# xujiabo/SCREAM

Hardware: AMD Instinct MI355X
Metric: registration pairs/sec (higher is better)
Workload: dtype f32; 1 GPU; BASELINE configs[1]: synthetic 3DMatch_test-like pairs, voxel 0.0625 m, ~5k points/cloud, batch-of-pairs=32 per GPU, A1-A10 per pair (forward 6+6 layers d_model 256, 1-NN thresh 0.1, Kabsch, RE/TE), random-init weights seed 0; lanes=1, steps_in_flight=2, parallelism=dp1 (pairs sharded, metric-row all-gather), rccl_ranks=1, gemm_backend=h2

## Files before the change

### scream_amd/csrc/proj_ring.hip

```cpp
#include <type_traits>

#include "matrix_front.h"
#include "ring.h"

namespace {

constexpr int P_PF = 2;
constexpr int P_LB = 2;

constexpr int P_KV_ELEMS = (SCREAM_HEAD_DIM + 1) * SCREAM_HEAD_DIM;
constexpr int P_SLAB_BYTES = 4 * P_KV_ELEMS * 4;

struct ProjArgs {
    const float* x;
    const char* Wimg;
    float* Q;
    int64_t M;
    int32_t n_q;
    int32_t S;
    float* kv_partial;
    int64_t kv_layer_stride;
    const int32_t* tile_cloud;
    const int32_t* cloud_row0;
    const int32_t* cloud_len;
    int64_t row_base;
    float a_scale, kv_sk, kv_cv, kv_inv;
    Elu1Consts ec;
};

template <class SP>
__global__ __launch_bounds__(TT, 1) void proj_ring_kernel(ProjArgs pa) {
    typedef typename SP::vec V;
    constexpr int NP = SP::NP;
    constexpr int STAGE = stage_bytes<SP>();
    constexpr int PIECES = wave_pieces<SP>();
    constexpr int INFLIGHT = PIECES;
    constexpr int GM = 2 * SP::NPROD;
    constexpr int Q_WIN = 12;
    constexpr int PIECE_STRIDE = (15 - Q_WIN) * GM / PIECES;
    static_assert(PIECE_STRIDE >= 1, "the groups behind the stores hold the stage's pieces");
    __shared__ __attribute__((aligned(16))) char smem[T_SLOTS * STAGE + P_SLAB_BYTES];
    float* slabs = reinterpret_cast<float*>(smem + T_SLOTS * STAGE);
    const int tid = threadIdx.x, lane = tid & 63;
    const int wave = __builtin_amdgcn_readfirstlane(tid >> 6);
    const int half = lane >> 5, r = lane & 31;
    const unsigned v_lane16 = lane * 16;

    const int S = pa.S, UPT = S >> 1, nq2 = pa.n_q >> 1;
    const int64_t n_tiles = (pa.M + 255) >> 8;
    const int64_t U = n_tiles * UPT;
    const int64_t u_lo = U * blockIdx.x / gridDim.x, u_hi = U * (blockIdx.x + 1) / gridDim.x;
    if (u_lo >= u_hi) return;
    const int s0 = (int)(u_lo % UPT) * 2;

    unsigned q = 0;
    auto dma_piece = [&](unsigned qq, int u) __attribute__((always_inline)) {
        const unsigned img = (unsigned)(s0 + qq) % (unsigned)S, slot = qq % (unsigned)T_SLOTS;
        const char* sbase = pa.Wimg + (size_t)img * STAGE + (wave * PIECES + (u & ~3)) * 1024;
        dma_1k(sbase + v_lane16, smem + slot * STAGE + (wave * PIECES + (u & ~3)) * 1024, u & 3);
    };
#pragma unroll
    for (int u = 0; u < PIECES; ++u) dma_piece(0, u);
#pragma unroll
    for (int u = 0; u < PIECES; ++u) dma_piece(1, u);

    V xp[2][16][NP];
    int64_t tile = -1;
    bool wave_ok = false;
    int valid0 = 0;
    float* part_tile = nullptr;
    float* qg = nullptr;

    auto enter_tile = [&](int64_t t) __attribute__((always_inline)) {
        tile = t;
        const int64_t t128 = t * 2 + (wave >> 1);
        wave_ok = t128 * 128 < pa.M;
        const int64_t row0 = wave_ok ? t * 256 + wave * 64 : t * 256;
        const float* g = pa.x + row0 * SCREAM_D_MODEL + lane * 4;
        valid0 = 0;
        if (wave_ok && pa.S > pa.n_q) {
            const int64_t arow = pa.row_base + t128 * 128;
            const int cloud = pa.tile_cloud[arow / SCREAM_ROW_TILE];
            valid0 = pa.cloud_len[cloud] - (int)(arow - pa.cloud_row0[cloud]) - (wave & 1) * 64;
        }
        part_tile = pa.kv_partial + t128 * SCREAM_NHEAD * P_KV_ELEMS;
        qg = pa.Q + row0 * SCREAM_D_MODEL + lane * 4;
        constexpr int LB = P_LB, NB = 16 / LB;
        f32x4 raw[2][LB][4];
        auto request = [&](int b) __attribute__((always_inline)) {
            const int rg = b / (NB / 2), blk0 = LB * (b % (NB / 2));
#pragma unroll
            for (int k = 0; k < LB; ++k)
#pragma unroll
                for (int a = 0; a < 4; ++a)
                    raw[b & 1][k][a] = __builtin_nontemporal_load(reinterpret_cast<const f32x4*>(g + rg * 8192 + ((blk0 + k) * 4 + a) * 256));
        };
        request(0);
#pragma unroll
        for (int b = 0; b < NB; ++b) {
            const int rg = b / (NB / 2), blk0 = LB * (b % (NB / 2));
            __builtin_amdgcn_sched_barrier(0);
            if (b + 1 < NB) request(b + 1);
            __builtin_amdgcn_sched_barrier(0);
#pragma unroll
            for (int k = 0; k < LB; ++k)
#pragma unroll
                for (int s2 = 0; s2 < 2; ++s2)
                {
                    V tmp[NP];
#pragma unroll
                    for (int j = 0; j < 8; ++j) SP::split1s(raw[b & 1][k][2 * s2 + (j >> 2)][j & 3], pa.a_scale, j, tmp);
#pragma unroll
                    for (int p = 0; p < NP; ++p) {
                        asm volatile("" : "+a"(tmp[p]));
                        xp[rg][2 * (blk0 + k) + s2][p] = tmp[p];
                    }
                }
        }
        __builtin_amdgcn_sched_barrier(0);
    };

    f32x16 acc[2][2];
    f16x8 kp[2][2][2];
    f32x16 kv;
    float ks = 0.f;
    float* q_pend = nullptr;
    bool q_pend_ok = false;
    float* part_pend = nullptr;
    bool part_pend_ok = false;

    auto stage = [&](auto kind, f32x16 (&a)[2], auto ride) __attribute__((always_inline)) {
        constexpr int KIND = decltype(kind)::value;
        ring_barrier<INFLIGHT>();
        __builtin_amdgcn_sched_barrier(0);
        const char* wb = smem + (q % T_SLOTS) * STAGE + lane * 16;
        V wf[P_PF][NP];
        f32x16 z;
#pragma unroll
        for (int e = 0; e < 16; ++e) z[e] = 0.f;
#pragma unroll
        for (int g0 = 0; g0 < P_PF - 1; ++g0)
#pragma unroll
            for (int p = 0; p < NP; ++p) wf[g0][p] = ld_frag<V>(wb + (p * 16 + g0) * 1024);
#pragma unroll
        for (int g = 0; g < 16; ++g) {
#pragma unroll
            for (int m = 0; m < GM; ++m) {
                const int rg = m / SP::NPROD, i = m % SP::NPROD;
                __builtin_amdgcn_sched_barrier(0);
                if (KIND == 0) a[rg] = SP::product(i, wf[g % P_PF], xp[rg][g], g == 0 && i == 0 ? z : a[rg]);
                else a[rg] = SP::product(i, xp[rg][g], wf[g % P_PF], g == 0 && i == 0 ? z : a[rg]);
                __builtin_amdgcn_sched_barrier(0);
                if (m == 0 && g + P_PF - 1 < 16) {
#pragma unroll
                    for (int p = 0; p < NP; ++p) wf[(g + P_PF - 1) % P_PF][p] = ld_frag<V>(wb + (p * 16 + g + P_PF - 1) * 1024);
                }
                const int ps = (g - Q_WIN - 1) * GM + m;
                if (ps >= 0 && ps % PIECE_STRIDE == 0 && ps / PIECE_STRIDE < PIECES) dma_piece(q + 2, ps / PIECE_STRIDE);
                ride(g, m);
            }
        }
        __builtin_amdgcn_sched_barrier(0);
        ++q;
    };
    static_assert(wave_pieces<SP>() <= 8, "the request schedule of a stage holds eight pieces");
    constexpr std::integral_constant<int, 0> kindQ{};
    constexpr std::integral_constant<int, 1> kindKV{};

    auto first_item = [](int s, int n_items, int n_slots) __attribute__((always_inline)) { return (s * n_items + n_slots - 1) / n_slots; };
    auto per_slot = [](int n_items, int n_slots) constexpr { return (n_items + n_slots - 1) / n_slots; };
    Elu1Pair ep;
    auto ride_q = [&](f32x16 (&t)[2], int g, int m) __attribute__((always_inline)) {
        if (g < Q_WIN) {
            const int s = g * GM + m;
#pragma unroll
            for (int j = 0; j < per_slot(64, Q_WIN * GM); ++j) {
                const int k = first_item(s, 64, Q_WIN * GM) + j;
                if (k < first_item(s + 1, 64, Q_WIN * GM)) elu1s_pair(k & 3, t[0], t[1], k >> 2, ep, pa.ec);
            }
        }
        if (g == Q_WIN && m == 0) {
            if (q_pend_ok) {
#pragma unroll
                for (int rg = 0; rg < 2; ++rg)
#pragma unroll
                    for (int a = 0; a < 4; ++a) {
                        const f32x4 o = {t[rg][4 * a], t[rg][4 * a + 1], t[rg][4 * a + 2], t[rg][4 * a + 3]};
                        __builtin_nontemporal_store(o, reinterpret_cast<f32x4*>(q_pend + rg * 8192 + a * 256));
                    }
            }
        }
    };
    auto ride_k = [&](auto mask, f32x16 (&t)[2], int valid, int g, int m) __attribute__((always_inline)) {
#pragma unroll
        for (int j = 0; j < per_slot(6, GM); ++j) {
            const int k = first_item(m, 6, GM) + j;
            if (k >= first_item(m + 1, 6, GM)) continue;
            if (k < 4) elu1s_pair(k, t[0], t[1], g, ep, pa.ec);
            if (k == 4) {
                if (g == 0) ks = 0.f;
#pragma unroll
                for (int rg = 0; rg < 2; ++rg) {
                    if (decltype(mask)::value && (g & 3) + 8 * (g >> 2) + 32 * rg >= valid) t[rg][g] = 0.f;
                    ks += t[rg][g];
                }
                keep_here(ks);
            }
            if (k == 5) {
                SplitH2::split1s_pair_here(t[0][g], t[1][g], pa.kv_sk, g & 7, kp[0][g >> 3], kp[1][g >> 3]);
                if (g == 15) ks += __shfl_xor(ks, 32);
            }
        }
    };
    f16x8 vp[2][2];
    auto ride_v = [&](const f32x16 (&t)[2], int g, int m) __attribute__((always_inline)) {
        if (g < 8) {
            const int s2 = g >> 2;
            if (m < 2) {
                const int i = 8 * s2 + 2 * (g & 3) + m;
                SplitH2::split1s_pair_here(t[0][i], t[1][i], pa.kv_cv, i & 7, vp[0], vp[1]);
            }
            if ((g & 3) == 3 && m == GM - 1) {
                f32x16 z;
#pragma unroll
                for (int e = 0; e < 16; ++e) z[e] = 0.f;
                SplitH2::products(kv, kp[0][s2], vp[0], s2 == 0 ? z : kv);
                SplitH2::products(kv, kp[1][s2], vp[1], kv);
            }
        }
        if (g == 9) {
#pragma unroll
            for (int j = 0; j < per_slot(16, GM); ++j) {
                const int e = first_item(m, 16, GM) + j;
                if (e < first_item(m + 1, 16, GM)) kv[e] *= pa.kv_inv;
            }
        }
        if (g >= 10 && g < 14) {
            float* sw = slabs + wave * P_KV_ELEMS;
            const int s = (g - 10) * GM + m;
#pragma unroll
            for (int j = 0; j < per_slot(16, 4 * GM); ++j) {
                const int e = first_item(s, 16, 4 * GM) + j;
                if (e < first_item(s + 1, 16, 4 * GM)) sw[mfma32_row(e, half) * 32 + r] = kv[e];
            }
            if (g == 13 && m == GM - 1 && half == 0) sw[32 * 32 + r] = ks;
        }
    };
    float kvs[2];
    auto ride_kvstore = [&](int g, int m) __attribute__((always_inline)) {
        constexpr int M_RD = GM >= 4 ? 1 : 0, M_ST = GM >= 4 ? 3 : GM - 1;
        if (g > 8 || (m != M_RD && m != M_ST)) return;
        const int i = (wave & 1) * 64 + lane + 128 * g;
        if (i < P_KV_ELEMS && part_pend_ok) {
            const float* s2 = slabs + (wave & ~1) * P_KV_ELEMS + i;
            if (m == M_RD) {
                kvs[0] = s2[0];
                kvs[1] = s2[P_KV_ELEMS];
            }
            if (m == M_ST) part_pend[i] = kvs[0] + kvs[1];
        }
    };

    int prev = 0;
    auto no_ride = [&](int, int) __attribute__((always_inline)) {};
#define LAMBDA(...) [&](__VA_ARGS__) __attribute__((always_inline))
    for (int64_t u = u_lo; u < u_hi; ++u) {
        const int64_t t = u / UPT;
        const int uu = (int)(u - t * UPT);
        if (t != tile) enter_tile(t);
        if (uu < nq2) {
            float* q_even = qg + (2 * uu) * 1024;
            if (prev == 0) stage(kindQ, acc[0], no_ride);
            else if (prev == 1) stage(kindQ, acc[0], LAMBDA(int g, int m) { ride_q(acc[1], g, m); });
            else stage(kindQ, acc[0], LAMBDA(int g, int m) { ride_v(acc[1], g, m); });
            const bool store_kv = prev == 2;
            q_pend = q_even;
            q_pend_ok = wave_ok;
            if (store_kv) stage(kindQ, acc[1], LAMBDA(int g, int m) { ride_kvstore(g, m); ride_q(acc[0], g, m); });
            else stage(kindQ, acc[1], LAMBDA(int g, int m) { ride_q(acc[0], g, m); });
            q_pend = q_even + 1024;
            prev = 1;
        } else {
            const int p = uu - nq2, l = p >> 3, h = p & 7;
            if (prev == 0) stage(kindKV, acc[0], no_ride);
            else if (prev == 1) stage(kindKV, acc[0], LAMBDA(int g, int m) { ride_q(acc[1], g, m); });
            else stage(kindKV, acc[0], LAMBDA(int g, int m) { ride_v(acc[1], g, m); });
            const bool store_kv = prev == 2;
            const int valid = valid0 - 4 * half;
            constexpr std::integral_constant<bool, true> masked{};
            constexpr std::integral_constant<bool, false> whole{};
            if (valid0 < 64) {
                if (store_kv) stage(kindKV, acc[1], LAMBDA(int g, int m) { ride_kvstore(g, m); ride_k(masked, acc[0], valid, g, m); });
                else stage(kindKV, acc[1], LAMBDA(int g, int m) { ride_k(masked, acc[0], valid, g, m); });
            } else {
                if (store_kv) stage(kindKV, acc[1], LAMBDA(int g, int m) { ride_kvstore(g, m); ride_k(whole, acc[0], valid, g, m); });
                else stage(kindKV, acc[1], LAMBDA(int g, int m) { ride_k(whole, acc[0], valid, g, m); });
            }
            part_pend = part_tile + (int64_t)l * pa.kv_layer_stride + h * P_KV_ELEMS;
            part_pend_ok = wave_ok;
            prev = 2;
        }
    }
    __builtin_amdgcn_sched_barrier(0);
    if (prev == 1) {
#pragma unroll
        for (int g = 0; g <= Q_WIN; ++g)
#pragma unroll
            for (int m = 0; m < GM; ++m) ride_q(acc[1], g, m);
    } else if (prev == 2) {
        lds_barrier();
#pragma unroll
        for (int g = 0; g < 14; ++g)
#pragma unroll
            for (int m = 0; m < GM; ++m) ride_v(acc[1], g, m);
        lds_barrier();
#pragma unroll
        for (int g = 0; g < 9; ++g)
#pragma unroll
            for (int m = 0; m < GM; ++m) ride_kvstore(g, m);
    }
#undef LAMBDA
    VM_WAIT(0);
}

template <class SP>
__global__ void pack_proj_kernel(const float* __restrict__ W, int n_q, int S, float w_scale, typename SP::vec* __restrict__ out) {
    const int t = blockIdx.x * blockDim.x + threadIdx.x;
    if (t >= S * 16 * 64) return;
    const int lane = t & 63, frag = (t >> 6) & 15, stage = t >> 10;
    const int m = lane & 31, half = lane >> 5;
    int row0;
    if (stage < n_q / 32) {
        row0 = 32 * stage;
    } else {
        const int st = stage - n_q / 32, p = st >> 1, l = p >> 3, h = p & 7, is_v = st & 1;
        row0 = n_q + l * 512 + (h >> 2) * 256 + is_v * 128 + (h & 3) * 32;
    }
    float v[8];
#pragma unroll
    for (int j = 0; j < 8; ++j) v[j] = W[(int64_t)(row0 + m) * 256 + 32 * (frag >> 1) + chunk_k(frag & 1, half, j)];
    typename SP::vec p[SP::NP];
#pragma unroll
    for (int j = 0; j < 8; ++j) SP::split1(v[j] * w_scale, j, p);
#pragma unroll
    for (int pl = 0; pl < SP::NP; ++pl) out[(((int64_t)stage * SP::NP + pl) * 16 + frag) * 64 + lane] = p[pl];
}

}

extern "C" int64_t scream_proj_image_bytes(int32_t N, int32_t split) {
    if (!split_fp16(split) || N <= 0 || N % 64 != 0) return SCREAM_EINVAL;
    return (int64_t)(N / 32) * split * 16 * 1024;
}

extern "C" int scream_pack_proj(const float* W, int32_t N, int32_t n_q, int32_t split, int32_t w_exp, void* image, void* stream) {
    SCREAM_REQUIRE(W && image && split_fp16(split), SCREAM_EINVAL);
    SCREAM_REQUIRE((n_q == 0 || n_q == SCREAM_D_MODEL) && N > n_q && (N - n_q) % 512 == 0, SCREAM_EUNSUPPORTED);
    SCREAM_REQUIRE(operand_exp_ok(w_exp) && aligned16(image), SCREAM_EINVAL);
    const int S = N / 32;
    const dim3 grid(S * 16 * 64 / 256), block(256);
    with_split(split, [&](auto tag) {
        typedef typename decltype(tag)::type SP;
        if constexpr (SP::SCALED)
            pack_proj_kernel<SP><<<grid, block, 0, as_stream(stream)>>>(W, n_q, S, exp2i(w_exp), reinterpret_cast<f16x8*>(image));
    });
    SCREAM_LAUNCH_CHECK();
    return 0;
}

extern "C" int scream_proj_qkv_f32(const float* x, const void* proj_image, float* Q, int64_t M, int32_t N, int32_t n_q,
                                   const int32_t* tile_cloud, const int32_t* cloud_row0, const int32_t* cloud_len,
                                   int64_t row_base, float* kv_partial, int32_t split, int32_t a_exp, int32_t w_exp, int32_t k_exp,
                                   int32_t v_exp, void* stream) {
    SCREAM_REQUIRE(split_fp16(split), SCREAM_EINVAL);
    if (int rc = check_qkv(x, SCREAM_D_MODEL, proj_image, Q, SCREAM_D_MODEL, M, N, SCREAM_D_MODEL, n_q, tile_cloud, cloud_row0, cloud_len,
                           row_base, kv_partial, K_64_PLUS_192, true))
        return rc;
    SCREAM_REQUIRE(proj_exps_ok(a_exp, w_exp, k_exp, v_exp), SCREAM_EINVAL);
    SCREAM_REQUIRE(aligned16(Q) && aligned16(kv_partial), SCREAM_EINVAL);
    if (M == 0) return 0;
    ProjArgs pa;
    pa.x = x;
    pa.Wimg = reinterpret_cast<const char*>(proj_image);
    pa.Q = Q;
    pa.M = M;
    pa.n_q = n_q / 32;
    pa.S = N / 32;
    pa.kv_partial = kv_partial;
    pa.kv_layer_stride = (M / SCREAM_ROW_TILE) * SCREAM_NHEAD * (int64_t)P_KV_ELEMS;
    pa.tile_cloud = tile_cloud;
    pa.cloud_row0 = cloud_row0;
    pa.cloud_len = cloud_len;
    pa.row_base = row_base;
    pa.a_scale = exp2i(a_exp);
    pa.ec = elu1_consts(exp2i(-a_exp - w_exp));
    pa.kv_sk = exp2i(k_exp);
    pa.kv_cv = exp2i(-a_exp - w_exp + v_exp);
    pa.kv_inv = exp2i(-k_exp - v_exp);
    const int grid = persistent_grid(((M + 255) / 256) * (pa.S / 2), SCREAM_MAX_GRID, false);
    with_split(split, [&](auto tag) {
        typedef typename decltype(tag)::type SP;
        if constexpr (SP::SCALED) proj_ring_kernel<SP><<<dim3(grid), dim3(TT), 0, as_stream(stream)>>>(pa);
    });
    SCREAM_LAUNCH_CHECK();
    return 0;
}
```

### scream_amd/csrc/ring.h

```cpp
#pragma once
#include "split.h"

namespace {

constexpr int T_PF = 3;

constexpr int TT = 256;
constexpr int T_SLOTS = 3;

template <class SP> constexpr int stage_bytes() { return SP::NP * 16 * 1024; }
template <class SP> constexpr int wave_pieces() { return SP::NP * 4; }

__host__ __device__ __forceinline__ int chunk_k(int s2, int half, int j) { return 8 * (2 * s2 + (j >> 2)) + 4 * half + (j & 3); }

__device__ __forceinline__ void dma_1k(const char* src_lane, char* dst, int k) {
    switch (k) {
        case 0: __builtin_amdgcn_global_load_lds((gptr_t)src_lane, (lptr_t)dst, 16, 0, 0); break;
        case 1: __builtin_amdgcn_global_load_lds((gptr_t)src_lane, (lptr_t)dst, 16, 1024, 0); break;
        case 2: __builtin_amdgcn_global_load_lds((gptr_t)src_lane, (lptr_t)dst, 16, 2048, 0); break;
        default: __builtin_amdgcn_global_load_lds((gptr_t)src_lane, (lptr_t)dst, 16, 3072, 0); break;
    }
}

template <class V>
__device__ __forceinline__ V ld_frag(const char* p) {
    return *reinterpret_cast<const V*>(p);
}

template <class SP, int NV = 0>
__device__ __forceinline__ void mfma_group(f32x16& acc, const typename SP::vec (&w)[SP::NP], const typename SP::vec (&a)[SP::NP],
                                           bool zero = false) {
    f32x16 z;
#pragma unroll
    for (int e = 0; e < 16; ++e) z[e] = 0.f;
    SP::products(acc, w, a, zero ? z : acc);
    if (NV < 0) return;
    __builtin_amdgcn_sched_group_barrier(0x008, 1, 0);
    __builtin_amdgcn_sched_group_barrier(0x100, SP::NP, 0);
    if (NV == 0) {
        if (SP::NPROD > 1) __builtin_amdgcn_sched_group_barrier(0x008, SP::NPROD - 1, 0);
    } else {
#pragma unroll
        for (int i = 0; i < SP::NPROD - 1; ++i) {
            __builtin_amdgcn_sched_group_barrier(0x002, NV, 0);
            __builtin_amdgcn_sched_group_barrier(0x008, 1, 0);
        }
        __builtin_amdgcn_sched_group_barrier(0x002, NV, 0);
    }
    __builtin_amdgcn_sched_barrier(0);
}

template <int STEP, bool NT = false>
__device__ __forceinline__ void ld_asm4(f32x4 (&d)[4], const void* sbase, unsigned voff) {
    static_assert(STEP == 1024 || STEP == 32, "");
    if (STEP == 1024 && NT) {
        asm volatile("global_load_dwordx4 %0, %1, %2 nt" : "=v"(d[0]) : "v"(voff), "s"(sbase));
        asm volatile("global_load_dwordx4 %0, %1, %2 offset:1024 nt" : "=v"(d[1]) : "v"(voff), "s"(sbase));
        asm volatile("global_load_dwordx4 %0, %1, %2 offset:2048 nt" : "=v"(d[2]) : "v"(voff), "s"(sbase));
        asm volatile("global_load_dwordx4 %0, %1, %2 offset:3072 nt" : "=v"(d[3]) : "v"(voff), "s"(sbase));
    } else if (STEP == 1024) {
        asm volatile("global_load_dwordx4 %0, %1, %2" : "=v"(d[0]) : "v"(voff), "s"(sbase));
        asm volatile("global_load_dwordx4 %0, %1, %2 offset:1024" : "=v"(d[1]) : "v"(voff), "s"(sbase));
        asm volatile("global_load_dwordx4 %0, %1, %2 offset:2048" : "=v"(d[2]) : "v"(voff), "s"(sbase));
        asm volatile("global_load_dwordx4 %0, %1, %2 offset:3072" : "=v"(d[3]) : "v"(voff), "s"(sbase));
    } else {
        asm volatile("global_load_dwordx4 %0, %1, %2" : "=v"(d[0]) : "v"(voff), "s"(sbase));
        asm volatile("global_load_dwordx4 %0, %1, %2 offset:32" : "=v"(d[1]) : "v"(voff), "s"(sbase));
        asm volatile("global_load_dwordx4 %0, %1, %2 offset:64" : "=v"(d[2]) : "v"(voff), "s"(sbase));
        asm volatile("global_load_dwordx4 %0, %1, %2 offset:96" : "=v"(d[3]) : "v"(voff), "s"(sbase));
    }
}
__device__ __forceinline__ void ld_asm2k(f32x4& d0, f32x4& d1, const void* sbase, unsigned voff) {
    asm volatile("global_load_dwordx4 %0, %1, %2" : "=v"(d0) : "v"(voff), "s"(sbase));
    asm volatile("global_load_dwordx4 %0, %1, %2 offset:1024" : "=v"(d1) : "v"(voff), "s"(sbase));
}
__device__ __forceinline__ void pin(f32x4& v) { asm volatile("" : "+v"(v)); }

#define VM_WAIT(N) asm volatile("s_waitcnt vmcnt(" #N ")" ::: "memory")
template <int N>
__device__ __forceinline__ void vm_wait() {
    static_assert(N == 0 || N == 4 || N == 8 || N == 12, "");
    if (N == 0) VM_WAIT(0);
    else if (N == 4) VM_WAIT(4);
    else if (N == 8) VM_WAIT(8);
    else VM_WAIT(12);
}

}
```

Baseline: 1905 pairs/s.

## Deepen activation prefetch window with explicit vmcnt-tracked asm loads in projection

Replaces the double-buffered nontemporal intrinsic loads of the activation tile with an 8-deep window of inline-asm global loads. Explicit per-step s_waitcnt vmcnt values let more memory requests stay in flight while earlier slices are split into MFMA operands. Adds split2s to convert pairs of elements at once, and reads the cloud lookup tables through the constant address space so they can become scalar loads. The trade-off is more live VGPRs for the raw window, which may lower occupancy. The code depends on v_lane16 and vm_wait ordering being correct with respect to other outstanding loads.

```diff
diff --git a/scream_amd/csrc/proj_ring.hip b/scream_amd/csrc/proj_ring.hip
--- a/scream_amd/csrc/proj_ring.hip
+++ b/scream_amd/csrc/proj_ring.hip
@@ -6,7 +6,8 @@
 namespace {
 
 constexpr int P_PF = 2;
-constexpr int P_LB = 2;
+
+constexpr int P_WIN = 8;
 
 constexpr int P_KV_ELEMS = (SCREAM_HEAD_DIM + 1) * SCREAM_HEAD_DIM;
 constexpr int P_SLAB_BYTES = 4 * P_KV_ELEMS * 4;
@@ -76,46 +77,45 @@
         const int64_t t128 = t * 2 + (wave >> 1);
         wave_ok = t128 * 128 < pa.M;
         const int64_t row0 = wave_ok ? t * 256 + wave * 64 : t * 256;
-        const float* g = pa.x + row0 * SCREAM_D_MODEL + lane * 4;
+        const char* xw = reinterpret_cast<const char*>(pa.x + row0 * SCREAM_D_MODEL);
         valid0 = 0;
         if (wave_ok && pa.S > pa.n_q) {
             const int64_t arow = pa.row_base + t128 * 128;
-            const int cloud = pa.tile_cloud[arow / SCREAM_ROW_TILE];
-            valid0 = pa.cloud_len[cloud] - (int)(arow - pa.cloud_row0[cloud]) - (wave & 1) * 64;
+            typedef const __attribute__((address_space(4))) int32_t* ctab;
+            const int cloud = ((ctab)pa.tile_cloud)[arow / SCREAM_ROW_TILE];
+            valid0 = ((ctab)pa.cloud_len)[cloud] - (int)(arow - ((ctab)pa.cloud_row0)[cloud]) - (wave & 1) * 64;
         }
         part_tile = pa.kv_partial + t128 * SCREAM_NHEAD * P_KV_ELEMS;
         qg = pa.Q + row0 * SCREAM_D_MODEL + lane * 4;
-        constexpr int LB = P_LB, NB = 16 / LB;
-        f32x4 raw[2][LB][4];
-        auto request = [&](int b) __attribute__((always_inline)) {
-            const int rg = b / (NB / 2), blk0 = LB * (b % (NB / 2));
-#pragma unroll
-            for (int k = 0; k < LB; ++k)
-#pragma unroll
-                for (int a = 0; a < 4; ++a)
-                    raw[b & 1][k][a] = __builtin_nontemporal_load(reinterpret_cast<const f32x4*>(g + rg * 8192 + ((blk0 + k) * 4 + a) * 256));
+        f32x4 raw[P_WIN][4];
+        auto request = [&](int s) __attribute__((always_inline)) {
+            ld_asm4<1024, true>(raw[s % P_WIN], xw + (s >> 3) * 32768 + (s & 7) * 4096, v_lane16);
         };
-        request(0);
-#pragma unroll
-        for (int b = 0; b < NB; ++b) {
-            const int rg = b / (NB / 2), blk0 = LB * (b % (NB / 2));
+        __builtin_amdgcn_sched_barrier(0);
+#pragma unroll
+        for (int s = 0; s < P_WIN; ++s) request(s);
+#pragma unroll
+        for (int s = 0; s < 16; ++s) {
+            const int rg = s >> 3, blk = s & 7;
             __builtin_amdgcn_sched_barrier(0);
-            if (b + 1 < NB) request(b + 1);
+            vm_wait_x4(15 - s < P_WIN - 1 ? 15 - s : P_WIN - 1);
+#pragma unroll
+            for (int a = 0; a < 4; ++a) pin(raw[s % P_WIN][a]);
             __builtin_amdgcn_sched_barrier(0);
 #pragma unroll
-            for (int k = 0; k < LB; ++k)
-#pragma unroll
-                for (int s2 = 0; s2 < 2; ++s2)
-                {
-                    V tmp[NP];
-#pragma unroll
-                    for (int j = 0; j < 8; ++j) SP::split1s(raw[b & 1][k][2 * s2 + (j >> 2)][j & 3], pa.a_scale, j, tmp);
-#pragma unroll
-                    for (int p = 0; p < NP; ++p) {
-                        asm volatile("" : "+a"(tmp[p]));
-                        xp[rg][2 * (blk0 + k) + s2][p] = tmp[p];
-                    }
+            for (int s2 = 0; s2 < 2; ++s2) {
+                V tmp[NP];
+#pragma unroll
+                for (int j = 0; j < 8; j += 2)
+                    SP::split2s(raw[s % P_WIN][2 * s2 + (j >> 2)][j & 3], raw[s % P_WIN][2 * s2 + (j >> 2)][(j & 3) + 1], pa.a_scale, j, tmp);
+#pragma unroll
+                for (int p = 0; p < NP; ++p) {
+                    asm volatile("" : "+a"(tmp[p]));
+                    xp[rg][2 * blk + s2][p] = tmp[p];
                 }
+            }
+            __builtin_amdgcn_sched_barrier(0);
+            if (s + P_WIN < 16) request(s + P_WIN);
         }
         __builtin_amdgcn_sched_barrier(0);
     };
diff --git a/scream_amd/csrc/ring.h b/scream_amd/csrc/ring.h
--- a/scream_amd/csrc/ring.h
+++ b/scream_amd/csrc/ring.h
@@ -77,6 +77,26 @@
 __device__ __forceinline__ void pin(f32x4& v) { asm volatile("" : "+v"(v)); }
 
 #define VM_WAIT(N) asm volatile("s_waitcnt vmcnt(" #N ")" ::: "memory")
+__device__ __forceinline__ void vm_wait_x4(int n4) {
+    switch (n4) {
+        case 0: VM_WAIT(0); break;
+        case 1: VM_WAIT(4); break;
+        case 2: VM_WAIT(8); break;
+        case 3: VM_WAIT(12); break;
+        case 4: VM_WAIT(16); break;
+        case 5: VM_WAIT(20); break;
+        case 6: VM_WAIT(24); break;
+        case 7: VM_WAIT(28); break;
+        case 8: VM_WAIT(32); break;
+        case 9: VM_WAIT(36); break;
+        case 10: VM_WAIT(40); break;
+        case 11: VM_WAIT(44); break;
+        case 12: VM_WAIT(48); break;
+        case 13: VM_WAIT(52); break;
+        case 14: VM_WAIT(56); break;
+        default: VM_WAIT(60); break;
+    }
+}
 template <int N>
 __device__ __forceinline__ void vm_wait() {
     static_assert(N == 0 || N == 4 || N == 8 || N == 12, "");
```

New measurement: 1911 pairs/s (median of 6 runs). Within noise of the previous version (+0.3%).
